# nkb-tech/nkb-classification

Measured on AMD Instinct MI355X. Metric: images/sec train step (3x224x224), higher is better.
Workload: dtype bf16; 1 GPU; resnet50 single-task train step, 1000 classes, bs=256/GPU, bf16 compute + fp32 master weights, NAdam, 3x224x224; global_batch=256, parallelism=dp1

## Files before the change

### nkb-classification_amd/csrc/elementwise.hip

```cpp
#include "common.h"
#include <stdlib.h>
#include <atomic>

static inline unsigned grid_for(size_t work_items, int block = 256, unsigned cap = 256 * 16) {
    size_t g = (work_items + block - 1) / block;
    if (g > cap) g = cap;
    if (g < 1) g = 1;
    return (unsigned)g;
}

template <typename T> struct Chunk;
template <> struct Chunk<bf16_t> {
    static constexpr int N = 8;
    __device__ static __forceinline__ void load(const bf16_t* p, float* f) { unpack8(*(const u32x4*)p, f); }
    __device__ static __forceinline__ void store(bf16_t* p, const float* f) { *(u32x4*)p = pack8(f); }
};
template <> struct Chunk<float> {
    static constexpr int N = 4;
    __device__ static __forceinline__ void load(const float* p, float* f) {
        const f32x4 v = *(const f32x4*)p;
        f[0] = v[0]; f[1] = v[1]; f[2] = v[2]; f[3] = v[3];
    }
    __device__ static __forceinline__ void store(float* p, const float* f) { *(f32x4*)p = (f32x4){f[0], f[1], f[2], f[3]}; }
};

static inline int env_int(const char* name, int dflt) {
    const char* v = getenv(name);
    return v && *v ? atoi(v) : dflt;
}
#ifndef NKB_BN_FUSED
#define NKB_BN_FUSED 1
#endif
static constexpr int g_bn_fused = NKB_BN_FUSED;

template <int NC>
__device__ __forceinline__ void ldvec(const float* __restrict__ p, float* o) {
#pragma unroll
    for (int i = 0; i < NC / 4; ++i) {
        const f32x4 v = *(const f32x4*)(p + 4 * i);
        o[4 * i] = v[0]; o[4 * i + 1] = v[1]; o[4 * i + 2] = v[2]; o[4 * i + 3] = v[3];
    }
}

static inline int bn_partitions(int C) { return C <= 128 ? 64 : (C <= 256 ? 32 : 16); }
template <bool WT>
__device__ __forceinline__ void bn_partial_reduce_body(const float* __restrict__ partials, int tiles, int C, double* __restrict__ dpart,
                                                       double (&red)[2][16][64]) {
    const int cx = threadIdx.x & 63, py = threadIdx.x >> 6;
    const int c = blockIdx.x * 64 + cx;
    double s = 0.0, ss = 0.0;
    if (c < C) {
        for (int t = blockIdx.y * 16 + py; t < tiles; t += 16 * (int)gridDim.y) {
            s += (double)partials[((size_t)t * 2) * C + c];
            ss += (double)partials[((size_t)t * 2 + 1) * C + c];
        }
    }
    red[0][py][cx] = s;
    red[1][py][cx] = ss;
    __syncthreads();
    if (py != 0 || c >= C) return;
    s = 0.0; ss = 0.0;
    for (int k = 0; k < 16; ++k) { s += red[0][k][cx]; ss += red[1][k][cx]; }
    double* d0 = dpart + ((size_t)blockIdx.y * 2) * C + c;
    double* d1 = dpart + ((size_t)blockIdx.y * 2 + 1) * C + c;
    if constexpr (WT) {
        __hip_atomic_store(d0, s, __ATOMIC_RELAXED, __HIP_MEMORY_SCOPE_AGENT);
        __hip_atomic_store(d1, ss, __ATOMIC_RELAXED, __HIP_MEMORY_SCOPE_AGENT);
    } else {
        *d0 = s; *d1 = ss;
    }
}
__global__ void bn_partial_reduce_kernel(const float* __restrict__ partials, int tiles, int C, double* __restrict__ dpart) {
    __shared__ double red[2][16][64];
    bn_partial_reduce_body<false>(partials, tiles, C, dpart, red);
}

__device__ unsigned g_bn_tickets[128 * 32];
__device__ __forceinline__ bool bn_arrive_last(unsigned* ticket, unsigned parts) {
    __shared__ unsigned last_flag;
    asm volatile("s_waitcnt vmcnt(0)" ::: "memory");
    __syncthreads();
    if (threadIdx.x == 0) {
        const unsigned t = __hip_atomic_fetch_add(ticket, 1u, __ATOMIC_RELAXED, __HIP_MEMORY_SCOPE_AGENT);
        const bool last = t == parts - 1;
        if (last) {
            __hip_atomic_store(ticket, 0u, __ATOMIC_RELAXED, __HIP_MEMORY_SCOPE_AGENT);
            __builtin_amdgcn_fence(__ATOMIC_ACQUIRE, "agent");
            asm volatile("s_waitcnt vmcnt(0)" ::: "memory");
        }
        last_flag = last ? 1u : 0u;
    }
    __syncthreads();
    return last_flag != 0u;
}
static unsigned* bn_ticket_slot(int cols) {
    static std::atomic<unsigned> next{0};
    if (cols > 32) return nullptr;
    unsigned* base = nullptr;
    if (hipGetSymbolAddress((void**)&base, HIP_SYMBOL(g_bn_tickets)) != hipSuccess || !base) return nullptr;
    return base + (next.fetch_add(1u) % 128u) * 32u;
}

template <typename PT>
__device__ __forceinline__ void bn_finalize_body(const PT* __restrict__ partials, int tiles, int C, float count,
                                                 const float* __restrict__ gamma, const float* __restrict__ beta,
                                                 float* __restrict__ running_mean, float* __restrict__ running_var,
                                                 float momentum, float eps, int training, float* __restrict__ scale,
                                                 float* __restrict__ shift, float* __restrict__ save_mean,
                                                 float* __restrict__ save_invstd, double (&red)[2][16][64]) {
    const int cx = threadIdx.x & 63, py = threadIdx.x >> 6;
    const int c = blockIdx.x * 64 + cx;
    double s = 0.0, ss = 0.0;
    if (training && c < C) {
        for (int t = py; t < tiles; t += 16) {
            s += (double)partials[((size_t)t * 2) * C + c];
            ss += (double)partials[((size_t)t * 2 + 1) * C + c];
        }
    }
    red[0][py][cx] = s;
    red[1][py][cx] = ss;
    __syncthreads();
    if (py != 0 || c >= C) return;
    float mean, var;
    if (training) {
        s = 0.0; ss = 0.0;
        for (int k = 0; k < 16; ++k) { s += red[0][k][cx]; ss += red[1][k][cx]; }
        const double m = s / count;
        double v = ss / count - m * m;
        if (v < 0.0) v = 0.0;
        mean = (float)m; var = (float)v;
        const float unbiased = count > 1.f ? (float)(v * count / (count - 1.0)) : var;
        running_mean[c] = (1.f - momentum) * running_mean[c] + momentum * mean;
        running_var[c] = (1.f - momentum) * running_var[c] + momentum * unbiased;
    } else {
        mean = running_mean[c]; var = running_var[c];
    }
    const float invstd = 1.0f / sqrtf(var + eps);
    const float g = gamma ? gamma[c] : 1.f, b = beta ? beta[c] : 0.f;
    scale[c] = g * invstd;
    shift[c] = b - mean * g * invstd;
    if (save_mean) { save_mean[c] = mean; save_invstd[c] = invstd; }
}
template <typename PT>
__global__ void bn_finalize_kernel(const PT* __restrict__ partials, int tiles, int C, float count,
                                   const float* __restrict__ gamma, const float* __restrict__ beta,
                                   float* __restrict__ running_mean, float* __restrict__ running_var,
                                   float momentum, float eps, int training, float* __restrict__ scale,
                                   float* __restrict__ shift, float* __restrict__ save_mean,
                                   float* __restrict__ save_invstd) {
    __shared__ double red[2][16][64];
    bn_finalize_body<PT>(partials, tiles, C, count, gamma, beta, running_mean, running_var, momentum, eps, training, scale, shift,
                         save_mean, save_invstd, red);
}
__global__ __launch_bounds__(1024) void bn_reduce_finalize_kernel(const float* __restrict__ partials, int tiles, int C, double* __restrict__ dpart,
                                                                  unsigned* __restrict__ tickets, float count,
                                                                  const float* __restrict__ gamma, const float* __restrict__ beta,
                                                                  float* __restrict__ running_mean, float* __restrict__ running_var,
                                                                  float momentum, float eps, float* __restrict__ scale,
                                                                  float* __restrict__ shift, float* __restrict__ save_mean,
                                                                  float* __restrict__ save_invstd) {
    __shared__ double red[2][16][64];
    bn_partial_reduce_body<true>(partials, tiles, C, dpart, red);
    if (!bn_arrive_last(tickets + blockIdx.x, gridDim.y)) return;
    bn_finalize_body<double>(dpart, (int)gridDim.y, C, count, gamma, beta, running_mean, running_var, momentum, eps, 1, scale, shift,
                             save_mean, save_invstd, red);
}

extern "C" int nkb_bn_finalize(const float* partials, int tiles, int C, long long count, const float* gamma,
                               const float* beta, float* running_mean, float* running_var, float momentum, float eps,
                               int training, float* scale, float* shift, float* save_mean, float* save_invstd,
                               hipStream_t stream) {
// ... 714 lines not shown
}
extern "C" int nkb_wprep(int dtype, const float* src, void* dst, int A, int B, int C, int ld, int mode, hipStream_t stream) {
    if (mode < 0 || mode > 5 || (mode >= 2 && B != 9)) { nkb_set_error("wprep: bad mode %d (B=%d)", mode, B); return 1; }
    const size_t total = wprep_total(A, B, C, ld, mode);
    NkbProfScope prof(NKB_K_WPREP, stream, 0);
    if (dtype == NKB_DT_BF16)
        hipLaunchKernelGGL(wprep_kernel<bf16_t>, dim3(grid_for(total)), dim3(256), 0, stream, src, (bf16_t*)dst, A, B, C, ld, mode, total);
    else
        hipLaunchKernelGGL(wprep_kernel<float>, dim3(grid_for(total)), dim3(256), 0, stream, src, (float*)dst, A, B, C, ld, mode, total);
    return nkb_check_launch("wprep");
}

template <typename T>
__global__ void wfold_kernel(const float* __restrict__ w, const float* __restrict__ scale, T* __restrict__ dst, int K, size_t total) {
    for (size_t i = (size_t)blockIdx.x * blockDim.x + threadIdx.x; i < total; i += (size_t)gridDim.x * blockDim.x)
        DT<T>::st(dst + i, w[i] * scale[i / K]);
}
extern "C" int nkb_wfold(int dtype, const float* w, const float* scale, void* dst, int Cout, int K, hipStream_t stream) {
    if (dtype != NKB_DT_BF16 && dtype != NKB_DT_F32) { nkb_set_error("wfold: bad dtype %d", dtype); return 1; }
    if (Cout <= 0 || K <= 0) return 0;
    const size_t total = (size_t)Cout * K;
    NkbProfScope prof(NKB_K_WPREP, stream, 0);
    if (dtype == NKB_DT_BF16) hipLaunchKernelGGL(wfold_kernel<bf16_t>, dim3(grid_for(total)), dim3(256), 0, stream, w, scale, (bf16_t*)dst, K, total);
    else hipLaunchKernelGGL(wfold_kernel<float>, dim3(grid_for(total)), dim3(256), 0, stream, w, scale, (float*)dst, K, total);
    return nkb_check_launch("wfold");
}

template <typename T>
__global__ void splitk_reduce_kernel(const float* __restrict__ partial, int S, int M, int N, T* __restrict__ y, int ldy,
                                     const float* __restrict__ bias, float* __restrict__ stats) {
    const int n = blockIdx.x * blockDim.x + threadIdx.x;
    if (n >= N) return;
    const int m0 = blockIdx.y * 128, m1 = min(M, m0 + 128);
    const float b = bias ? bias[n] : 0.f;
    float s = 0.f, ss = 0.f;
    for (int m = m0; m < m1; ++m) {
        float v = b;
        for (int z = 0; z < S; ++z) v += partial[((size_t)z * M + m) * N + n];
        v = DT<T>::rnd(v);
        DT<T>::st(y + (size_t)m * ldy + n, v);
        s += v; ss += v * v;
    }
    if (stats) {
        stats[((size_t)blockIdx.y * 2) * N + n] = s;
        stats[((size_t)blockIdx.y * 2 + 1) * N + n] = ss;
    }
}
template <typename T>
__global__ void splitk_reduce4_kernel(const float* __restrict__ partial, int S, int M, int N, T* __restrict__ y, int ldy,
                                      const float* __restrict__ bias) {
    const int n4 = N >> 2;
    const size_t i = (size_t)blockIdx.x * blockDim.x + threadIdx.x;
    if (i >= (size_t)M * n4) return;
    const int m = (int)(i / n4), c = (int)(i - (size_t)m * n4) * 4;
    f32x4 v = bias ? *(const f32x4*)(bias + c) : (f32x4){0.f, 0.f, 0.f, 0.f};
    const float* p = partial + (size_t)m * N + c;
    const size_t slab = (size_t)M * N;
    for (int z = 0; z < S; ++z) v += *(const f32x4*)(p + (size_t)z * slab);
#pragma unroll
    for (int e = 0; e < 4; ++e) DT<T>::st(y + (size_t)m * ldy + c + e, DT<T>::rnd(v[e]));
}
template <typename T>
__global__ void splitk_stats_kernel(const T* __restrict__ y, int M, int N, int ldy, float* __restrict__ stats) {
    const int n = blockIdx.x * blockDim.x + threadIdx.x;
    if (n >= N) return;
    const int m0 = blockIdx.y * 128, m1 = min(M, m0 + 128);
    float s = 0.f, ss = 0.f;
    for (int m = m0; m < m1; ++m) { const float v = DT<T>::ld(y + (size_t)m * ldy + n); s += v; ss += v * v; }
    stats[((size_t)blockIdx.y * 2) * N + n] = s;
    stats[((size_t)blockIdx.y * 2 + 1) * N + n] = ss;
}
extern "C" int nkb_splitk_reduce(int dtype, const float* partial, int splits, int M, int N, void* y, int ldy, const float* bias,
                                 float* stats, hipStream_t stream) {
    if (dtype != NKB_DT_BF16 && dtype != NKB_DT_F32) { nkb_set_error("splitk_reduce: bad dtype %d", dtype); return 1; }
    if (splits < 1 || M < 1 || N < 1 || ldy < N) { nkb_set_error("splitk_reduce: bad shape"); return 1; }
    NkbProfScope prof(NKB_K_MISC, stream, 0);
    if (N % 4 == 0 && (((size_t)bias) & 15) == 0) {
        const size_t total = (size_t)M * (N >> 2);
        const dim3 g4((unsigned)((total + 255) / 256)), gs((N + 255) / 256, (M + 127) / 128);
        if (dtype == NKB_DT_BF16) {
            hipLaunchKernelGGL(splitk_reduce4_kernel<bf16_t>, g4, dim3(256), 0, stream, partial, splits, M, N, (bf16_t*)y, ldy, bias);
            if (stats) hipLaunchKernelGGL(splitk_stats_kernel<bf16_t>, gs, dim3(256), 0, stream, (const bf16_t*)y, M, N, ldy, stats);
        } else {
            hipLaunchKernelGGL(splitk_reduce4_kernel<float>, g4, dim3(256), 0, stream, partial, splits, M, N, (float*)y, ldy, bias);
            if (stats) hipLaunchKernelGGL(splitk_stats_kernel<float>, gs, dim3(256), 0, stream, (const float*)y, M, N, ldy, stats);
        }
        return nkb_check_launch("splitk_reduce");
    }
    dim3 grid((N + 255) / 256, (M + 127) / 128);
    if (dtype == NKB_DT_BF16) hipLaunchKernelGGL(splitk_reduce_kernel<bf16_t>, grid, dim3(256), 0, stream, partial, splits, M, N, (bf16_t*)y, ldy, bias, stats);
    else hipLaunchKernelGGL(splitk_reduce_kernel<float>, grid, dim3(256), 0, stream, partial, splits, M, N, (float*)y, ldy, bias, stats);
    return nkb_check_launch("splitk_reduce");
}

__global__ void add2d_kernel(const float* __restrict__ src, float* __restrict__ dst, int rows, int cols, int ld_src, int ld_dst) {
    const size_t total = (size_t)rows * cols;
    for (size_t i = (size_t)blockIdx.x * blockDim.x + threadIdx.x; i < total; i += (size_t)gridDim.x * blockDim.x) {
        const int c = (int)(i % cols), r = (int)(i / cols);
        dst[(size_t)r * ld_dst + c] += src[(size_t)r * ld_src + c];
    }
}
extern "C" int nkb_add2d(const float* src, float* dst, int rows, int cols, int ld_src, int ld_dst, hipStream_t stream) {
    NkbProfScope prof(NKB_K_MISC, stream, 0);
    hipLaunchKernelGGL(add2d_kernel, dim3(grid_for((size_t)rows * cols)), dim3(256), 0, stream, src, dst, rows, cols, ld_src, ld_dst);
    return nkb_check_launch("add2d");
}

template <typename T>
__global__ void colsum_kernel(const T* __restrict__ x, float* __restrict__ out, int rows, int C, int ld) {
    const int c = blockIdx.x * 64 + (threadIdx.x & 63);
    const int part = threadIdx.x >> 6;
    __shared__ float red[4][64];
    float t = 0.f;
    if (c < C) for (int r = part; r < rows; r += 4) t += DT<T>::ld(x + (size_t)r * ld + c);
    red[part][threadIdx.x & 63] = t;
    __syncthreads();
    if (part == 0 && c < C) out[c] += red[0][threadIdx.x] + red[1][threadIdx.x] + red[2][threadIdx.x] + red[3][threadIdx.x];
}
extern "C" int nkb_colsum(int dtype, const void* x, float* out, int rows, int C, int ld, hipStream_t stream) {
    NkbProfScope prof(NKB_K_MISC, stream, 0);
    if (dtype == NKB_DT_BF16) hipLaunchKernelGGL(colsum_kernel<bf16_t>, dim3((C + 63) / 64), dim3(256), 0, stream, (const bf16_t*)x, out, rows, C, ld);
    else hipLaunchKernelGGL(colsum_kernel<float>, dim3((C + 63) / 64), dim3(256), 0, stream, (const float*)x, out, rows, C, ld);
    return nkb_check_launch("colsum");
}

template <typename T>
__global__ void pad_cast_kernel(const float* __restrict__ src, T* __restrict__ dst, int rows, int C, int ld_src, int ld_dst, float mul) {
    const size_t total = (size_t)rows * ld_dst;
    for (size_t i = (size_t)blockIdx.x * blockDim.x + threadIdx.x; i < total; i += (size_t)gridDim.x * blockDim.x) {
        const int c = (int)(i % ld_dst), r = (int)(i / ld_dst);
        DT<T>::st(dst + i, c < C ? src[(size_t)r * ld_src + c] * mul : 0.f);
    }
}
extern "C" int nkb_pad_cast(int dtype, const float* src, void* dst, int rows, int C, int ld_src, int ld_dst, float mul, hipStream_t stream) {
    NkbProfScope prof(NKB_K_MISC, stream, 0);
    const size_t total = (size_t)rows * ld_dst;
    if (dtype == NKB_DT_BF16) hipLaunchKernelGGL(pad_cast_kernel<bf16_t>, dim3(grid_for(total)), dim3(256), 0, stream, src, (bf16_t*)dst, rows, C, ld_src, ld_dst, mul);
    else hipLaunchKernelGGL(pad_cast_kernel<float>, dim3(grid_for(total)), dim3(256), 0, stream, src, (float*)dst, rows, C, ld_src, ld_dst, mul);
    return nkb_check_launch("pad_cast");
}

template <int NC> struct SlotWord;
template <> struct SlotWord<8> {
    unsigned long long w;
    __device__ __forceinline__ void load(const unsigned char* p) { w = *(const unsigned long long*)p; }
    __device__ __forceinline__ int get(int e) const { return (int)((w >> (8 * e)) & 0xff); }
};
template <> struct SlotWord<4> {
    unsigned w;
    __device__ __forceinline__ void load(const unsigned char* p) { w = *(const unsigned*)p; }
    __device__ __forceinline__ int get(int e) const { return (int)((w >> (8 * e)) & 0xff); }
};

template <typename T>
__global__ __launch_bounds__(256) void bn_relu_maxpool_fwd_kernel(const T* __restrict__ c, const float* __restrict__ scale,
                                                                  const float* __restrict__ shift, T* __restrict__ y,
                                                                  unsigned char* __restrict__ idx, T* __restrict__ xsel, int N,
                                                                  int H, int W, int C, int P, int Q) {
    constexpr int NC = Chunk<T>::N;
    const unsigned cpr = (unsigned)C / NC;
    const unsigned t = blockIdx.x * blockDim.x + threadIdx.x;
    const unsigned cg = t % cpr, pstride = (gridDim.x * blockDim.x) / cpr;
    const unsigned npix = (unsigned)N * P * Q;
    float sc[NC], sh[NC];
    ldvec<NC>(scale + cg * NC, sc);
    ldvec<NC>(shift + cg * NC, sh);
    for (unsigned pix = t / cpr; pix < npix; pix += pstride) {
        const unsigned q = pix % (unsigned)Q, pn = pix / (unsigned)Q;
        const unsigned pp = pn % (unsigned)P, n = pn / (unsigned)P;
        float best[NC], bx[NC];
        int bi[NC];
#pragma unroll
        for (int e = 0; e < NC; ++e) { best[e] = -INFINITY; bi[e] = 0; bx[e] = 0.f; }
        bool first = true;
        for (int r = 0; r < 3; ++r) {
            const int h = 2 * (int)pp - 1 + r;
            if ((unsigned)h >= (unsigned)H) continue;
            for (int s = 0; s < 3; ++s) {
                const int w = 2 * (int)q - 1 + s;
                if ((unsigned)w >= (unsigned)W) continue;
                float v[NC];
                Chunk<T>::load(c + (((size_t)n * H + h) * W + w) * C + cg * NC, v);
#pragma unroll
                for (int e = 0; e < NC; ++e) {
                    const float a = DT<T>::rnd(fmaxf(v[e] * sc[e] + sh[e], 0.f));
                    if (first || a > best[e] || a != a) { best[e] = a; bi[e] = r * 3 + s; bx[e] = v[e]; }
                }
                first = false;
            }
        }
        const size_t o = (size_t)pix * C + cg * NC;
        Chunk<T>::store(y + o, best);
        if (xsel) Chunk<T>::store(xsel + o, bx);
        unsigned long long word = 0;
#pragma unroll
        for (int e = 0; e < NC; ++e) word |= (unsigned long long)bi[e] << (8 * e);
        if (NC == 8) *(unsigned long long*)(idx + o) = word;
        else *(unsigned*)(idx + o) = (unsigned)word;
    }
}

template <typename T>
__global__ void bn_relu_maxpool_bwd_reduce_kernel(const T* __restrict__ g, const unsigned char* __restrict__ idx,
                                                  const T* __restrict__ c, const float* __restrict__ scale,
                                                  const float* __restrict__ shift, const float* __restrict__ mean,
                                                  const float* __restrict__ invstd, const T* __restrict__ xsel, int N, int H,
                                                  int W, int C, int P, int Q, int rpb, float* __restrict__ part) {
    constexpr int NC = Chunk<T>::N;
    extern __shared__ float red[];
    const int cpr = C / NC;
    const int tpc = blockDim.x / cpr;
    const int cg = threadIdx.x % cpr, rl = threadIdx.x / cpr;
    float s1[NC], s2[NC];
#pragma unroll
    for (int e = 0; e < NC; ++e) { s1[e] = 0.f; s2[e] = 0.f; }
    const long long rows = (long long)N * P * Q;
    if (rl < tpc) {
        float sc[NC], sh[NC], mu[NC], is[NC];
        ldvec<NC>(scale + cg * NC, sc);
        ldvec<NC>(shift + cg * NC, sh);
        ldvec<NC>(mean + cg * NC, mu);
        ldvec<NC>(invstd + cg * NC, is);
        for (long long r = (long long)blockIdx.x * tpc + rl; r < rows; r += (long long)gridDim.x * tpc) {
            const unsigned ru = (unsigned)r;
            const int q = (int)(ru % (unsigned)Q);
            const unsigned pn = ru / (unsigned)Q;
            const int pp = (int)(pn % (unsigned)P);
            const int n = (int)(pn / (unsigned)P);
            const size_t o = (size_t)r * C + cg * NC;
            float gv[NC];
            Chunk<T>::load(g + o, gv);
            SlotWord<NC> sw;
            sw.load(idx + o);
            const T* cbase = c + (((size_t)n * H + (2 * pp - 1)) * W + (2 * q - 1)) * C + cg * NC;
            float xs[NC];
            if (xsel) Chunk<T>::load(xsel + o, xs);
#pragma unroll
            for (int e = 0; e < NC; ++e) {
                float x;
                if (xsel) x = xs[e];
                else {
                    const int slot = sw.get(e);
                    const int dr = (slot * 11) >> 5;
                    const int ds = slot - 3 * dr;
                    x = DT<T>::ld(cbase + ((ptrdiff_t)dr * W + ds) * C + e);
                }
                if (DT<T>::rnd(x * sc[e] + sh[e]) > 0.f) { s1[e] += gv[e]; s2[e] += gv[e] * (x - mu[e]) * is[e]; }
            }
        }
#pragma unroll
        for (int e = 0; e < NC; ++e) {
            red[(0 * tpc + rl) * C + cg * NC + e] = s1[e];
            red[(1 * tpc + rl) * C + cg * NC + e] = s2[e];
        }
    }
    __syncthreads();
    for (int i = threadIdx.x; i < 2 * C; i += blockDim.x) {
        const int which = i / C, ch = i % C;
        float t = 0.f;
        for (int k = 0; k < tpc; ++k) t += red[(which * tpc + k) * C + ch];
        part[((size_t)blockIdx.x * 2 + which) * C + ch] = t;
    }
}

template <typename T>
__global__ __launch_bounds__(256) void bn_relu_maxpool_bwd_apply_kernel(
    const T* __restrict__ g, const unsigned char* __restrict__ idx, const T* __restrict__ c,
    const float* __restrict__ scale, const float* __restrict__ shift, const float* __restrict__ mean,
    const float* __restrict__ invstd, const float* __restrict__ gamma, const float* __restrict__ sums, float inv_count,
    T* __restrict__ dc, int N, int H, int W, int C, int P, int Q) {
    constexpr int NC = Chunk<T>::N;
    const unsigned cpr = (unsigned)C / NC;
    const unsigned t = blockIdx.x * blockDim.x + threadIdx.x;
    const unsigned cg = t % cpr, pstride = (gridDim.x * blockDim.x) / cpr;
    const unsigned npix = (unsigned)N * H * W;
    float k1[NC], k2[NC], k3[NC], fs[NC], fb[NC], v_is[NC], v_ga[NC], v_mu[NC], v_s1[NC], v_s2[NC];
    ldvec<NC>(scale + cg * NC, fs);
    ldvec<NC>(shift + cg * NC, fb);
    ldvec<NC>(invstd + cg * NC, v_is);
    ldvec<NC>(mean + cg * NC, v_mu);
    ldvec<NC>(sums + cg * NC, v_s1);
    ldvec<NC>(sums + C + cg * NC, v_s2);
    if (gamma) ldvec<NC>(gamma + cg * NC, v_ga);
#pragma unroll
    for (int e = 0; e < NC; ++e) {
        const float is = v_is[e], ga = gamma ? v_ga[e] : 1.f, mu = v_mu[e];
        const float a = ga * is;
        const float sdy = v_s1[e] * inv_count, sdyx = v_s2[e] * inv_count;
        k1[e] = a;
        k2[e] = -a * is * sdyx;
        k3[e] = -a * sdy + a * is * sdyx * mu;
    }
    for (unsigned pix = t / cpr; pix < npix; pix += pstride) {
        const unsigned w = pix % (unsigned)W, hn = pix / (unsigned)W;
        const unsigned h = hn % (unsigned)H, n = hn / (unsigned)H;
        float acc[NC], xv[NC], out[NC];
        const size_t ofs = (size_t)pix * C + cg * NC;
        Chunk<T>::load(c + ofs, xv);
#pragma unroll
        for (int e = 0; e < NC; ++e) acc[e] = 0.f;
        const int p0 = h >> 1, p1 = (h + 1) >> 1, q0 = w >> 1, q1 = (w + 1) >> 1;
        float gv[4][NC];
        SlotWord<NC> sw[4];
        int slot[4];
        bool ok[4];
#pragma unroll
        for (int k = 0; k < 4; ++k) {
            const int pp = (k >> 1) ? p1 : p0, q = (k & 1) ? q1 : q0;
            ok[k] = pp < P && q < Q && !((k >> 1) && p1 == p0) && !((k & 1) && q1 == q0);
            const int pc = pp < P ? pp : P - 1, qc = q < Q ? q : Q - 1;
            slot[k] = ((int)h - (2 * pp - 1)) * 3 + ((int)w - (2 * q - 1));
            const size_t o = ((((size_t)n * P + pc) * Q + qc) * C) + cg * NC;
            Chunk<T>::load(g + o, gv[k]);
            sw[k].load(idx + o);
        }
#pragma unroll
        for (int k = 0; k < 4; ++k)
#pragma unroll
            for (int e = 0; e < NC; ++e) if (ok[k] && sw[k].get(e) == slot[k]) acc[e] += gv[k][e];
#pragma unroll
        for (int e = 0; e < NC; ++e) {
            float gg = acc[e];
            if (!(DT<T>::rnd(xv[e] * fs[e] + fb[e]) > 0.f)) gg = 0.f;
            out[e] = k1[e] * gg + (k2[e] * xv[e] + k3[e]);
        }
        Chunk<T>::store(dc + ofs, out);
    }
}

extern "C" int nkb_bn_relu_maxpool_sel(int dtype, int backward, const void* c, const float* scale, const float* shift,
                                       const float* mean, const float* invstd, const float* gamma, void* y_or_g,
                                       unsigned char* idx, void* dc, float* dgamma, float* dbeta, float* workspace,
                                       size_t workspace_floats, void* xsel, int N, int H, int W, int C, hipStream_t stream);
extern "C" int nkb_bn_relu_maxpool(int dtype, int backward, const void* c, const float* scale, const float* shift,
                                   const float* mean, const float* invstd, const float* gamma, void* y_or_g,
                                   unsigned char* idx, void* dc, float* dgamma, float* dbeta, float* workspace,
                                   size_t workspace_floats, int N, int H, int W, int C, hipStream_t stream) {
    return nkb_bn_relu_maxpool_sel(dtype, backward, c, scale, shift, mean, invstd, gamma, y_or_g, idx, dc, dgamma, dbeta, workspace,
                                   workspace_floats, nullptr, N, H, W, C, stream);
}
extern "C" int nkb_bn_relu_maxpool_sel(int dtype, int backward, const void* c, const float* scale, const float* shift,
                                       const float* mean, const float* invstd, const float* gamma, void* y_or_g,
                                       unsigned char* idx, void* dc, float* dgamma, float* dbeta, float* workspace,
                                       size_t workspace_floats, void* xsel, int N, int H, int W, int C, hipStream_t stream) {
    const int P = (H + 2 - 3) / 2 + 1, Q = (W + 2 - 3) / 2 + 1;
    const int n = dtype == NKB_DT_BF16 ? 8 : 4;
    if (C % n || C / n > 256) { nkb_set_error("bn_relu_maxpool: unsupported C=%d", C); return 1; }
    if ((long long)N * H * W >= (1ll << 31)) { nkb_set_error("bn_relu_maxpool: N*H*W too large"); return 1; }
    if (!backward) {
        NkbProfScope prof(NKB_K_MAXPOOL, stream, 0);
        const unsigned grid = grid_cols((size_t)N * P * Q, C / n);
        if (dtype == NKB_DT_BF16)
            hipLaunchKernelGGL(bn_relu_maxpool_fwd_kernel<bf16_t>, dim3(grid), dim3(256), 0, stream,
                               (const bf16_t*)c, scale, shift, (bf16_t*)y_or_g, idx, (bf16_t*)xsel, N, H, W, C, P, Q);
        else
            hipLaunchKernelGGL(bn_relu_maxpool_fwd_kernel<float>, dim3(grid), dim3(256), 0, stream,
                               (const float*)c, scale, shift, (float*)y_or_g, idx, (float*)xsel, N, H, W, C, P, Q);
        return nkb_check_launch("bn_relu_maxpool_fwd");
    }
    const long long rows = (long long)N * P * Q;
    const int cpr = C / n;
    const int tpc = 256 / cpr;
    int blocks = (int)((rows + 63) / 64);
    if (blocks > 1024) blocks = 1024;
    if (blocks < 1) blocks = 1;
    const int rpb = (int)((rows + blocks - 1) / blocks);
    blocks = (int)((rows + rpb - 1) / rpb);
    const size_t need = (size_t)blocks * 2 * C + 2 * C;
    if (workspace_floats < need) { nkb_set_error("bn_relu_maxpool: workspace %zu < %zu floats", workspace_floats, need); return 1; }
    float* part = workspace;
    float* sums = workspace + (size_t)blocks * 2 * C;
    const size_t lds = (size_t)2 * tpc * C * sizeof(float);
    {
        NkbProfScope prof(NKB_K_BN_BWD_REDUCE, stream, 0);
        if (dtype == NKB_DT_BF16)
            hipLaunchKernelGGL(bn_relu_maxpool_bwd_reduce_kernel<bf16_t>, dim3(blocks), dim3(256), lds, stream,
                               (const bf16_t*)y_or_g, idx, (const bf16_t*)c, scale, shift, mean, invstd, (const bf16_t*)xsel, N, H, W, C, P, Q,
                               rpb, part);
        else
            hipLaunchKernelGGL(bn_relu_maxpool_bwd_reduce_kernel<float>, dim3(blocks), dim3(256), lds, stream,
                               (const float*)y_or_g, idx, (const float*)c, scale, shift, mean, invstd, (const float*)xsel, N, H, W, C, P, Q,
                               rpb, part);
        hipLaunchKernelGGL(bn_bwd_finalize_kernel, dim3((C + 15) / 16), dim3(1024), 0, stream, part, blocks, C, dgamma, dbeta, sums);
    }
    if (int rc = nkb_check_launch("bn_relu_maxpool_bwd_reduce")) return rc;
    {
        NkbProfScope prof(NKB_K_BN_BWD_APPLY, stream, 0);
        const unsigned grid = grid_cols((size_t)N * H * W, cpr);
        const float inv_count = 1.0f / (float)((long long)N * H * W);
        if (dtype == NKB_DT_BF16)
            hipLaunchKernelGGL(bn_relu_maxpool_bwd_apply_kernel<bf16_t>, dim3(grid), dim3(256), 0, stream,
                               (const bf16_t*)y_or_g, idx, (const bf16_t*)c, scale, shift, mean, invstd, gamma, sums, inv_count,
                               (bf16_t*)dc, N, H, W, C, P, Q);
        else
            hipLaunchKernelGGL(bn_relu_maxpool_bwd_apply_kernel<float>, dim3(grid), dim3(256), 0, stream,
                               (const float*)y_or_g, idx, (const float*)c, scale, shift, mean, invstd, gamma, sums, inv_count,
                               (float*)dc, N, H, W, C, P, Q);
    }
    return nkb_check_launch("bn_relu_maxpool_bwd_apply");
}

extern "C" size_t nkb_bn_relu_maxpool_workspace_floats(int N, int H, int W, int C) {
    const long long P = (H + 2 - 3) / 2 + 1, Q = (W + 2 - 3) / 2 + 1;
    long long blocks = ((long long)N * P * Q + 63) / 64;
    if (blocks > 1024) blocks = 1024;
    if (blocks < 1) blocks = 1;
    return (size_t)blocks * 2 * C + 2 * C;
}

template <typename T>
__global__ void stem_pack_kernel(const float* __restrict__ x, T* __restrict__ out, int N, int C, int H, int W, int Wp) {
    const size_t total = (size_t)N * H * Wp;
    for (size_t i = (size_t)blockIdx.x * blockDim.x + threadIdx.x; i < total; i += (size_t)gridDim.x * blockDim.x) {
        const int w = (int)(i % Wp);
        const size_t nh = i / Wp;
        const size_t n = nh / H, h = nh - n * H;
        float v[4] = {0.f, 0.f, 0.f, 0.f};
        if (w < W)
            for (int c = 0; c < C; ++c) v[c] = x[((n * C + c) * H + h) * W + w];
        if constexpr (sizeof(T) == 2) {
            u32x2 o = {pack_bf2(v[0], v[1]), pack_bf2(v[2], v[3])};
            *(u32x2*)(out + i * 4) = o;
        } else {
            *(f32x4*)(out + i * 4) = (f32x4){v[0], v[1], v[2], v[3]};
        }
    }
}
extern "C" int nkb_stem_pack(int dtype, const float* x, void* out, int N, int C, int H, int W, hipStream_t stream) {
    if (C < 1 || C > 4) { nkb_set_error("stem_pack: C=%d outside 1..4", C); return 1; }
    NkbProfScope prof(NKB_K_IM2COL, stream, 0);
    const int Wp = (W + 1) & ~1;
    const size_t total = (size_t)N * H * Wp;
    if (dtype == NKB_DT_BF16) hipLaunchKernelGGL(stem_pack_kernel<bf16_t>, dim3(grid_for(total)), dim3(256), 0, stream, x, (bf16_t*)out, N, C, H, W, Wp);
    else hipLaunchKernelGGL(stem_pack_kernel<float>, dim3(grid_for(total)), dim3(256), 0, stream, x, (float*)out, N, C, H, W, Wp);
    return nkb_check_launch("stem_pack");
}

__device__ __forceinline__ bool stem_col_to_tap(int col, int epc, int cprw, int lead, int& r, int& s, int& ch) {
    const int j = col % epc, sc = (col / epc) % cprw;
    r = col / (epc * cprw);
    s = sc * (epc / 4) + j / 4 - lead;
    ch = j % 4;
    return r < 7 && s >= 0 && s < 7;
}
template <typename T>
__global__ void stem_weight_kernel(const float* __restrict__ src, T* __restrict__ wp, float* __restrict__ dw, int Cout,
                                   int C, int cols, int epc, int cprw, int lead, int fold) {
    const int total = Cout * cols;
    for (int i = blockIdx.x * blockDim.x + threadIdx.x; i < total; i += gridDim.x * blockDim.x) {
        const int co = i / cols, col = i - co * cols;
        int r, s, ch;
        const bool ok = stem_col_to_tap(col, epc, cprw, lead, r, s, ch) && ch < C;
        const int widx = ((co * 7 + r) * 7 + s) * C + ch;
        if (fold) { if (ok) dw[widx] += src[i]; }
        else DT<T>::st(wp + i, ok ? src[widx] : 0.f);
    }
}
extern "C" int nkb_stem_wprep(int dtype, const float* w, void* wp, int Cout, int C, hipStream_t stream) {
    const int epc = dtype == NKB_DT_BF16 ? 8 : 4, cprw = dtype == NKB_DT_BF16 ? 4 : 8, lead = dtype == NKB_DT_BF16 ? 1 : 0;
    const int rpt = 8 / cprw, cols = (7 + rpt - 1) / rpt * 8 * epc;
    NkbProfScope prof(NKB_K_WPREP, stream, 0);
    if (dtype == NKB_DT_BF16) hipLaunchKernelGGL(stem_weight_kernel<bf16_t>, dim3(grid_for((size_t)Cout * cols)), dim3(256), 0, stream, w, (bf16_t*)wp, nullptr, Cout, C, cols, epc, cprw, lead, 0);
    else hipLaunchKernelGGL(stem_weight_kernel<float>, dim3(grid_for((size_t)Cout * cols)), dim3(256), 0, stream, w, (float*)wp, nullptr, Cout, C, cols, epc, cprw, lead, 0);
    return nkb_check_launch("stem_wprep");
}
extern "C" int nkb_stem_wfold(int dtype, const float* dwp, float* dw, int Cout, int C, hipStream_t stream) {
    const int epc = dtype == NKB_DT_BF16 ? 8 : 4, cprw = dtype == NKB_DT_BF16 ? 4 : 8, lead = dtype == NKB_DT_BF16 ? 1 : 0;
    const int cols = 7 * cprw * epc;
    NkbProfScope prof(NKB_K_MISC, stream, 0);
    hipLaunchKernelGGL(stem_weight_kernel<float>, dim3(grid_for((size_t)Cout * cols)), dim3(256), 0, stream, dwp, nullptr, dw, Cout, C, cols, epc, cprw, lead, 1);
    return nkb_check_launch("stem_wfold");
}

template <typename PT>
__device__ __forceinline__ void bn_bwd_finalize_tiles_body(const PT* __restrict__ partials, int tiles, int C,
                                                           const float* __restrict__ invstd, float* __restrict__ dgamma,
                                                           float* __restrict__ dbeta, float* __restrict__ sums, double (&red)[2][16][64]) {
    const int cx = threadIdx.x & 63, py = threadIdx.x >> 6;
    const int c = blockIdx.x * 64 + cx;
    double a = 0.0, b = 0.0;
    if (c < C) {
        for (int t = py; t < tiles; t += 16) {
            a += (double)partials[((size_t)t * 2) * C + c];
            b += (double)partials[((size_t)t * 2 + 1) * C + c];
        }
    }
    red[0][py][cx] = a;
    red[1][py][cx] = b;
    __syncthreads();
    if (py != 0 || c >= C) return;
    a = 0.0; b = 0.0;
    for (int k = 0; k < 16; ++k) { a += red[0][k][cx]; b += red[1][k][cx]; }
    const float sg = (float)a, sgx = (float)(b * (invstd ? (double)invstd[c] : 1.0));
    sums[c] = sg;
    sums[C + c] = sgx;
    if (dbeta) dbeta[c] += sg;
    if (dgamma) dgamma[c] += sgx;
}
template <typename PT>
__global__ void bn_bwd_finalize_tiles_kernel(const PT* __restrict__ partials, int tiles, int C,
                                             const float* __restrict__ invstd, float* __restrict__ dgamma,
                                             float* __restrict__ dbeta, float* __restrict__ sums) {
    __shared__ double red[2][16][64];
    bn_bwd_finalize_tiles_body<PT>(partials, tiles, C, invstd, dgamma, dbeta, sums, red);
}
__global__ __launch_bounds__(1024) void bn_bwd_reduce_finalize_kernel(const float* __restrict__ stats, int tiles, int C, double* __restrict__ dpart,
                                                                      unsigned* __restrict__ tickets, const float* __restrict__ invstd,
                                                                      float* __restrict__ dgamma, float* __restrict__ dbeta,
                                                                      float* __restrict__ sums) {
    __shared__ double red[2][16][64];
    bn_partial_reduce_body<true>(stats, tiles, C, dpart, red);
    if (!bn_arrive_last(tickets + blockIdx.x, gridDim.y)) return;
    bn_bwd_finalize_tiles_body<double>(dpart, (int)gridDim.y, C, invstd, dgamma, dbeta, sums, red);
}

static void launch_bwd_tile_sums(float* stats, int tiles, int C, const float* invstd, float* dgamma, float* dbeta, float* sums,
                                 hipStream_t stream) {
    double* dpart = (double*)(stats + (((size_t)tiles * 2 * C + 1) & ~(size_t)1));
    const int P = bn_partitions(C);
    unsigned* tickets = g_bn_fused ? bn_ticket_slot((C + 63) / 64) : nullptr;
    if (tickets) {
        hipLaunchKernelGGL(bn_bwd_reduce_finalize_kernel, dim3((C + 63) / 64, P), dim3(1024), 0, stream, stats, tiles, C, dpart, tickets,
                           invstd, dgamma, dbeta, sums);
        return;
    }
    hipLaunchKernelGGL(bn_partial_reduce_kernel, dim3((C + 63) / 64, P), dim3(1024), 0, stream, stats, tiles, C, dpart);
    hipLaunchKernelGGL(bn_bwd_finalize_tiles_kernel<double>, dim3((C + 63) / 64), dim3(1024), 0, stream,
                       (const double*)dpart, P, C, invstd, dgamma, dbeta, sums);
}

int nkb_launch_tile_sums(float* stats, int tiles, int C, float* sums, hipStream_t stream) {
    if (tiles > 128) {
        launch_bwd_tile_sums(stats, tiles, C, nullptr, nullptr, nullptr, sums, stream);
    } else {
        hipLaunchKernelGGL(bn_bwd_finalize_tiles_kernel<float>, dim3((C + 63) / 64), dim3(1024), 0, stream,
                           (const float*)stats, tiles, C, (const float*)nullptr, (float*)nullptr, (float*)nullptr, sums);
    }
    return nkb_check_launch("tile_sums");
}

extern "C" int nkb_bn_backward_from_stats(int dtype, const void* g, const void* x, float* stats, int tiles,
                                          const float* mean, const float* invstd, const float* gamma, long long rows,
                                          int C, float* dgamma, float* dbeta, void* dx, float* sums, hipStream_t stream) {
    const int n = dtype == NKB_DT_BF16 ? 8 : 4;
    if (C % n || rows >= (1ll << 31)) { nkb_set_error("bn_backward_from_stats: unsupported C=%d / rows", C); return 1; }
    {
        NkbProfScope prof(NKB_K_BN_BWD_REDUCE, stream, 0);
        if (tiles > 128) {
            launch_bwd_tile_sums(stats, tiles, C, invstd, dgamma, dbeta, sums, stream);
        } else {
            hipLaunchKernelGGL(bn_bwd_finalize_tiles_kernel<float>, dim3((C + 63) / 64), dim3(1024), 0, stream,
                               (const float*)stats, tiles, C, invstd, dgamma, dbeta, sums);
        }
    }
    if (int rc = nkb_check_launch("bn_bwd_finalize_tiles")) return rc;
    NkbProfScope prof(NKB_K_BN_BWD_APPLY, stream, 0, (double)rows * C * (dtype == NKB_DT_BF16 ? 2 : 4) * 3);
    const unsigned grid = grid_cols((size_t)rows, C / n);
    if (dtype == NKB_DT_BF16)
        hipLaunchKernelGGL(bn_bwd_apply_kernel<bf16_t>, dim3(grid), dim3(256), 0, stream, (const bf16_t*)g, (const bf16_t*)x,
                           (const bf16_t*)nullptr, (const unsigned char*)nullptr, (const float*)nullptr, (const float*)nullptr, mean, invstd, gamma, sums,
                           1.0f / (float)rows, (unsigned)rows, C, (bf16_t*)dx, (bf16_t*)nullptr);
    else
        hipLaunchKernelGGL(bn_bwd_apply_kernel<float>, dim3(grid), dim3(256), 0, stream, (const float*)g, (const float*)x,
                           (const float*)nullptr, (const unsigned char*)nullptr, (const float*)nullptr, (const float*)nullptr, mean, invstd, gamma, sums,
                           1.0f / (float)rows, (unsigned)rows, C, (float*)dx, (float*)nullptr);
    return nkb_check_launch("bn_bwd_apply");
}
```

Measured before the change: 15410 images/sec.

## Band stem maxpool forward, block-wise pool backward, and pair-wise stem pack

The fused BN+ReLU+maxpool forward now has each thread handle a vertical band of output rows. Input rows shared between neighbouring pooling windows are reused from registers instead of being reloaded. The backward apply kernel now iterates over 2x2 input blocks per output pixel, loading each gradient and index once and writing four outputs, rather than gathering up to four neighbours per input pixel. Stem pack processes two pixels per thread using paired loads and wider stores. The trade-offs are more register pressure and fewer parallel work items in the forward pass.

```diff
diff --git a/nkb-classification_amd/csrc/elementwise.hip b/nkb-classification_amd/csrc/elementwise.hip
--- a/nkb-classification_amd/csrc/elementwise.hip
+++ b/nkb-classification_amd/csrc/elementwise.hip
@@ -12,11 +12,17 @@
 template <typename T> struct Chunk;
 template <> struct Chunk<bf16_t> {
     static constexpr int N = 8;
+    typedef u32x4 Raw;
+    __device__ static __forceinline__ Raw ldraw(const bf16_t* p) { return *(const u32x4*)p; }
+    __device__ static __forceinline__ void unpack(const Raw& r, float* f) { unpack8(r, f); }
     __device__ static __forceinline__ void load(const bf16_t* p, float* f) { unpack8(*(const u32x4*)p, f); }
     __device__ static __forceinline__ void store(bf16_t* p, const float* f) { *(u32x4*)p = pack8(f); }
 };
 template <> struct Chunk<float> {
     static constexpr int N = 4;
+    typedef f32x4 Raw;
+    __device__ static __forceinline__ Raw ldraw(const float* p) { return *(const f32x4*)p; }
+    __device__ static __forceinline__ void unpack(const Raw& r, float* f) { f[0] = r[0]; f[1] = r[1]; f[2] = r[2]; f[3] = r[3]; }
     __device__ static __forceinline__ void load(const float* p, float* f) {
         const f32x4 v = *(const f32x4*)p;
         f[0] = v[0]; f[1] = v[1]; f[2] = v[2]; f[3] = v[3];
@@ -1037,51 +1043,99 @@
     __device__ __forceinline__ int get(int e) const { return (int)((w >> (8 * e)) & 0xff); }
 };
 
+#ifndef NKB_STEM_BAND
+#define NKB_STEM_BAND 7
+#endif
+template <typename T> struct PoolRow { typename Chunk<T>::Raw v[3]; };
+template <typename T>
+__device__ __forceinline__ void pool_row_load(const T* __restrict__ row, int w0, int w1, int w2, int C, PoolRow<T>& r) {
+    r.v[0] = Chunk<T>::ldraw(row + (size_t)w0 * C);
+    r.v[1] = Chunk<T>::ldraw(row + (size_t)w1 * C);
+    r.v[2] = Chunk<T>::ldraw(row + (size_t)w2 * C);
+}
+template <typename T>
+__device__ __forceinline__ void pool_row_winner(const PoolRow<T>& r, bool ok0, bool ok2, const float* sc, const float* sh, float* a,
+                                                float* x, int* s) {
+    constexpr int NC = Chunk<T>::N;
+    float v[3][NC];
+#pragma unroll
+    for (int k = 0; k < 3; ++k) Chunk<T>::unpack(r.v[k], v[k]);
+#pragma unroll
+    for (int e = 0; e < NC; ++e) {
+        const float a0 = DT<T>::rnd(fmaxf(v[0][e] * sc[e] + sh[e], 0.f));
+        const float a1 = DT<T>::rnd(fmaxf(v[1][e] * sc[e] + sh[e], 0.f));
+        const float a2 = DT<T>::rnd(fmaxf(v[2][e] * sc[e] + sh[e], 0.f));
+        const bool t1 = !ok0 | (a1 > a0) | (a1 != a1);
+        const float b1 = t1 ? a1 : a0;
+        const bool t2 = ok2 & ((a2 > b1) | (a2 != a2));
+        a[e] = t2 ? a2 : b1;
+        x[e] = t2 ? v[2][e] : (t1 ? v[1][e] : v[0][e]);
+        s[e] = t2 ? 2 : (int)t1;
+    }
+}
+
 template <typename T>
 __global__ __launch_bounds__(256) void bn_relu_maxpool_fwd_kernel(const T* __restrict__ c, const float* __restrict__ scale,
                                                                   const float* __restrict__ shift, T* __restrict__ y,
                                                                   unsigned char* __restrict__ idx, T* __restrict__ xsel, int N,
                                                                   int H, int W, int C, int P, int Q) {
     constexpr int NC = Chunk<T>::N;
+    constexpr int BAND = NKB_STEM_BAND;
     const unsigned cpr = (unsigned)C / NC;
     const unsigned t = blockIdx.x * blockDim.x + threadIdx.x;
-    const unsigned cg = t % cpr, pstride = (gridDim.x * blockDim.x) / cpr;
-    const unsigned npix = (unsigned)N * P * Q;
+    const unsigned cg = t % cpr, istride = (gridDim.x * blockDim.x) / cpr;
+    const unsigned nbands = ((unsigned)P + BAND - 1) / BAND;
+    const unsigned nitems = (unsigned)N * nbands * (unsigned)Q;
     float sc[NC], sh[NC];
     ldvec<NC>(scale + cg * NC, sc);
     ldvec<NC>(shift + cg * NC, sh);
-    for (unsigned pix = t / cpr; pix < npix; pix += pstride) {
-        const unsigned q = pix % (unsigned)Q, pn = pix / (unsigned)Q;
-        const unsigned pp = pn % (unsigned)P, n = pn / (unsigned)P;
-        float best[NC], bx[NC];
-        int bi[NC];
-#pragma unroll
-        for (int e = 0; e < NC; ++e) { best[e] = -INFINITY; bi[e] = 0; bx[e] = 0.f; }
-        bool first = true;
-        for (int r = 0; r < 3; ++r) {
-            const int h = 2 * (int)pp - 1 + r;
-            if ((unsigned)h >= (unsigned)H) continue;
-            for (int s = 0; s < 3; ++s) {
-                const int w = 2 * (int)q - 1 + s;
-                if ((unsigned)w >= (unsigned)W) continue;
-                float v[NC];
-                Chunk<T>::load(c + (((size_t)n * H + h) * W + w) * C + cg * NC, v);
-#pragma unroll
-                for (int e = 0; e < NC; ++e) {
-                    const float a = DT<T>::rnd(fmaxf(v[e] * sc[e] + sh[e], 0.f));
-                    if (first || a > best[e] || a != a) { best[e] = a; bi[e] = r * 3 + s; bx[e] = v[e]; }
-                }
-                first = false;
+    for (unsigned item = t / cpr; item < nitems; item += istride) {
+        const unsigned q = item % (unsigned)Q, bn = item / (unsigned)Q;
+        const unsigned band = bn % nbands, n = bn / nbands;
+        const int p0 = (int)band * BAND, p1 = p0 + BAND < P ? p0 + BAND : P;
+        const bool ok0 = q > 0, ok2 = 2 * (int)q + 1 < W;
+        const int w1 = 2 * (int)q, w0 = ok0 ? w1 - 1 : w1, w2 = ok2 ? w1 + 1 : w1;
+        const T* img = c + (size_t)n * H * W * C + cg * NC;
+        const size_t rowlen = (size_t)W * C;
+        PoolRow<T> ra, rb, rc;
+        pool_row_load(img + (size_t)(p0 > 0 ? 2 * p0 - 1 : 0) * rowlen, w0, w1, w2, C, ra);
+        pool_row_load(img + (size_t)(2 * p0) * rowlen, w0, w1, w2, C, rb);
+        pool_row_load(img + (size_t)(2 * p0 + 1 < H ? 2 * p0 + 1 : H - 1) * rowlen, w0, w1, w2, C, rc);
+        float ta[NC], tx[NC];
+        int ts[NC];
+        pool_row_winner<T>(ra, ok0, ok2, sc, sh, ta, tx, ts);
+        for (int p = p0; p < p1; ++p) {
+            PoolRow<T> nb = rb, nc = rc;
+            if (p + 1 < p1) {
+                pool_row_load(img + (size_t)(2 * p + 2) * rowlen, w0, w1, w2, C, nb);
+                pool_row_load(img + (size_t)(2 * p + 3 < H ? 2 * p + 3 : H - 1) * rowlen, w0, w1, w2, C, nc);
             }
-        }
-        const size_t o = (size_t)pix * C + cg * NC;
-        Chunk<T>::store(y + o, best);
-        if (xsel) Chunk<T>::store(xsel + o, bx);
-        unsigned long long word = 0;
-#pragma unroll
-        for (int e = 0; e < NC; ++e) word |= (unsigned long long)bi[e] << (8 * e);
-        if (NC == 8) *(unsigned long long*)(idx + o) = word;
-        else *(unsigned*)(idx + o) = (unsigned)word;
+            float ma[NC], mx[NC], la[NC], lx[NC], best[NC], bx[NC];
+            int ms[NC], ls[NC];
+            pool_row_winner<T>(rb, ok0, ok2, sc, sh, ma, mx, ms);
+            pool_row_winner<T>(rc, ok0, ok2, sc, sh, la, lx, ls);
+            const bool okt = p > 0, okl = 2 * p + 1 < H;
+            unsigned long long word = 0;
+#pragma unroll
+            for (int e = 0; e < NC; ++e) {
+                const bool t1 = !okt | (ma[e] > ta[e]) | (ma[e] != ma[e]);
+                const float b1 = t1 ? ma[e] : ta[e];
+                const bool t2 = okl & ((la[e] > b1) | (la[e] != la[e]));
+                best[e] = t2 ? la[e] : b1;
+                bx[e] = t2 ? lx[e] : (t1 ? mx[e] : tx[e]);
+                const int m3 = 3 + ms[e], l6 = 6 + ls[e];
+                const int b1i = t1 ? m3 : ts[e];
+                const int bi = t2 ? l6 : b1i;
+                word |= (unsigned long long)bi << (8 * e);
+                ta[e] = la[e]; tx[e] = lx[e]; ts[e] = ls[e];
+            }
+            const size_t o = ((((size_t)n * P + p) * Q + q) * C) + cg * NC;
+            Chunk<T>::store(y + o, best);
+            if (xsel) Chunk<T>::store(xsel + o, bx);
+            if (NC == 8) *(unsigned long long*)(idx + o) = word;
+            else *(unsigned*)(idx + o) = (unsigned)word;
+            rb = nb; rc = nc;
+        }
     }
 }
 
@@ -1157,8 +1211,8 @@
     constexpr int NC = Chunk<T>::N;
     const unsigned cpr = (unsigned)C / NC;
     const unsigned t = blockIdx.x * blockDim.x + threadIdx.x;
-    const unsigned cg = t % cpr, pstride = (gridDim.x * blockDim.x) / cpr;
-    const unsigned npix = (unsigned)N * H * W;
+    const unsigned cg = t % cpr, bstride = (gridDim.x * blockDim.x) / cpr;
+    const unsigned nblk = (unsigned)N * P * Q;
     float k1[NC], k2[NC], k3[NC], fs[NC], fb[NC], v_is[NC], v_ga[NC], v_mu[NC], v_s1[NC], v_s2[NC];
     ldvec<NC>(scale + cg * NC, fs);
     ldvec<NC>(shift + cg * NC, fb);
@@ -1176,40 +1230,49 @@
         k2[e] = -a * is * sdyx;
         k3[e] = -a * sdy + a * is * sdyx * mu;
     }
-    for (unsigned pix = t / cpr; pix < npix; pix += pstride) {
-        const unsigned w = pix % (unsigned)W, hn = pix / (unsigned)W;
-        const unsigned h = hn % (unsigned)H, n = hn / (unsigned)H;
-        float acc[NC], xv[NC], out[NC];
-        const size_t ofs = (size_t)pix * C + cg * NC;
-        Chunk<T>::load(c + ofs, xv);
-#pragma unroll
-        for (int e = 0; e < NC; ++e) acc[e] = 0.f;
-        const int p0 = h >> 1, p1 = (h + 1) >> 1, q0 = w >> 1, q1 = (w + 1) >> 1;
+    for (unsigned blk = t / cpr; blk < nblk; blk += bstride) {
+        const unsigned q = blk % (unsigned)Q, pn = blk / (unsigned)Q;
+        const unsigned p = pn % (unsigned)P, n = pn / (unsigned)P;
+        const int h0 = 2 * (int)p, w0 = 2 * (int)q;
+        const bool row1 = h0 + 1 < H, col1 = w0 + 1 < W;
+        const bool okp = (int)p + 1 < P, okq = (int)q + 1 < Q;
+        const size_t x0 = ((((size_t)n * H + h0) * W + w0) * C) + cg * NC, g0 = (size_t)blk * C + cg * NC;
+        const unsigned xstep[2] = {col1 ? (unsigned)C : 0u, row1 ? (unsigned)W * C : 0u};
+        const unsigned gstep[2] = {okq ? (unsigned)C : 0u, okp ? (unsigned)Q * C : 0u};
+        typename Chunk<T>::Raw xr[4], gr[4];
+        SlotWord<NC> sw[4];
+#pragma unroll
+        for (int k = 0; k < 4; ++k) {
+            xr[k] = Chunk<T>::ldraw(c + x0 + (k & 1) * xstep[0] + (k >> 1) * xstep[1]);
+            const size_t o = g0 + (k & 1) * gstep[0] + (k >> 1) * gstep[1];
+            gr[k] = Chunk<T>::ldraw(g + o);
+            sw[k].load(idx + o);
+        }
+        __builtin_amdgcn_sched_barrier(0);
+        const bool okw[4] = {true, okq, okp, okp && okq};
         float gv[4][NC];
-        SlotWord<NC> sw[4];
-        int slot[4];
-        bool ok[4];
-#pragma unroll
-        for (int k = 0; k < 4; ++k) {
-            const int pp = (k >> 1) ? p1 : p0, q = (k & 1) ? q1 : q0;
-            ok[k] = pp < P && q < Q && !((k >> 1) && p1 == p0) && !((k & 1) && q1 == q0);
-            const int pc = pp < P ? pp : P - 1, qc = q < Q ? q : Q - 1;
-            slot[k] = ((int)h - (2 * pp - 1)) * 3 + ((int)w - (2 * q - 1));
-            const size_t o = ((((size_t)n * P + pc) * Q + qc) * C) + cg * NC;
-            Chunk<T>::load(g + o, gv[k]);
-            sw[k].load(idx + o);
-        }
-#pragma unroll
-        for (int k = 0; k < 4; ++k)
-#pragma unroll
-            for (int e = 0; e < NC; ++e) if (ok[k] && sw[k].get(e) == slot[k]) acc[e] += gv[k][e];
-#pragma unroll
-        for (int e = 0; e < NC; ++e) {
-            float gg = acc[e];
-            if (!(DT<T>::rnd(xv[e] * fs[e] + fb[e]) > 0.f)) gg = 0.f;
-            out[e] = k1[e] * gg + (k2[e] * xv[e] + k3[e]);
-        }
-        Chunk<T>::store(dc + ofs, out);
+#pragma unroll
+        for (int k = 0; k < 4; ++k) Chunk<T>::unpack(gr[k], gv[k]);
+#pragma unroll
+        for (int k = 3; k >= 0; --k) {
+            const int dh = k >> 1, dw = k & 1;
+            float xv[NC], out[NC];
+            Chunk<T>::unpack(xr[k], xv);
+#pragma unroll
+            for (int e = 0; e < NC; ++e) {
+                float gg = 0.f;
+#pragma unroll
+                for (int j = 0; j < 4; ++j) {
+                    const int jp = j >> 1, jq = j & 1;
+                    if ((jp && !dh) || (jq && !dw)) continue;
+                    const int r = dh ? (jp ? 0 : 2) : 1, s = dw ? (jq ? 0 : 2) : 1;
+                    if (okw[j] && sw[j].get(e) == 3 * r + s) gg += gv[j][e];
+                }
+                if (!(DT<T>::rnd(xv[e] * fs[e] + fb[e]) > 0.f)) gg = 0.f;
+                out[e] = k1[e] * gg + (k2[e] * xv[e] + k3[e]);
+            }
+            Chunk<T>::store(dc + x0 + (k & 1) * xstep[0] + (k >> 1) * xstep[1], out);
+        }
     }
 }
 
@@ -1234,7 +1297,8 @@
     if ((long long)N * H * W >= (1ll << 31)) { nkb_set_error("bn_relu_maxpool: N*H*W too large"); return 1; }
     if (!backward) {
         NkbProfScope prof(NKB_K_MAXPOOL, stream, 0);
-        const unsigned grid = grid_cols((size_t)N * P * Q, C / n);
+        const size_t nbands = (size_t)(P + NKB_STEM_BAND - 1) / NKB_STEM_BAND;
+        const unsigned grid = grid_cols((size_t)N * nbands * Q, C / n, 16384);
         if (dtype == NKB_DT_BF16)
             hipLaunchKernelGGL(bn_relu_maxpool_fwd_kernel<bf16_t>, dim3(grid), dim3(256), 0, stream,
                                (const bf16_t*)c, scale, shift, (bf16_t*)y_or_g, idx, (bf16_t*)xsel, N, H, W, C, P, Q);
@@ -1271,7 +1335,7 @@
     if (int rc = nkb_check_launch("bn_relu_maxpool_bwd_reduce")) return rc;
     {
         NkbProfScope prof(NKB_K_BN_BWD_APPLY, stream, 0);
-        const unsigned grid = grid_cols((size_t)N * H * W, cpr);
+        const unsigned grid = grid_cols((size_t)N * P * Q, cpr);
         const float inv_count = 1.0f / (float)((long long)N * H * W);
         if (dtype == NKB_DT_BF16)
             hipLaunchKernelGGL(bn_relu_maxpool_bwd_apply_kernel<bf16_t>, dim3(grid), dim3(256), 0, stream,
@@ -1295,19 +1359,29 @@
 
 template <typename T>
 __global__ void stem_pack_kernel(const float* __restrict__ x, T* __restrict__ out, int N, int C, int H, int W, int Wp) {
-    const size_t total = (size_t)N * H * Wp;
+    const int Wh = Wp / 2;
+    const size_t total = (size_t)N * H * Wh;
+    const bool even = (W & 1) == 0;
     for (size_t i = (size_t)blockIdx.x * blockDim.x + threadIdx.x; i < total; i += (size_t)gridDim.x * blockDim.x) {
-        const int w = (int)(i % Wp);
-        const size_t nh = i / Wp;
+        const int w = 2 * (int)(i % Wh);
+        const size_t nh = i / Wh;
         const size_t n = nh / H, h = nh - n * H;
-        float v[4] = {0.f, 0.f, 0.f, 0.f};
-        if (w < W)
-            for (int c = 0; c < C; ++c) v[c] = x[((n * C + c) * H + h) * W + w];
+        float v[8] = {0.f, 0.f, 0.f, 0.f, 0.f, 0.f, 0.f, 0.f};
+        for (int c = 0; c < C; ++c) {
+            const float* src = x + ((n * C + c) * H + h) * W + w;
+            if (even) {
+                const nkb_f2 two = *(const nkb_f2*)src;
+                v[c] = two[0]; v[4 + c] = two[1];
+            } else {
+                v[c] = src[0];
+                if (w + 1 < W) v[4 + c] = src[1];
+            }
+        }
         if constexpr (sizeof(T) == 2) {
-            u32x2 o = {pack_bf2(v[0], v[1]), pack_bf2(v[2], v[3])};
-            *(u32x2*)(out + i * 4) = o;
+            *(u32x4*)(out + i * 8) = pack8(v);
         } else {
-            *(f32x4*)(out + i * 4) = (f32x4){v[0], v[1], v[2], v[3]};
+            *(f32x4*)(out + i * 8) = (f32x4){v[0], v[1], v[2], v[3]};
+            *(f32x4*)(out + i * 8 + 4) = (f32x4){v[4], v[5], v[6], v[7]};
         }
     }
 }
@@ -1315,7 +1389,7 @@
     if (C < 1 || C > 4) { nkb_set_error("stem_pack: C=%d outside 1..4", C); return 1; }
     NkbProfScope prof(NKB_K_IM2COL, stream, 0);
     const int Wp = (W + 1) & ~1;
-    const size_t total = (size_t)N * H * Wp;
+    const size_t total = (size_t)N * H * (Wp / 2);
     if (dtype == NKB_DT_BF16) hipLaunchKernelGGL(stem_pack_kernel<bf16_t>, dim3(grid_for(total)), dim3(256), 0, stream, x, (bf16_t*)out, N, C, H, W, Wp);
     else hipLaunchKernelGGL(stem_pack_kernel<float>, dim3(grid_for(total)), dim3(256), 0, stream, x, (float*)out, N, C, H, W, Wp);
     return nkb_check_launch("stem_pack");
```

New measurement: 15570 images/sec, median of 6. +1.0%, better.
